# TravisWheelerLab/AvxWindowFmIndex

Measured on AMD Instinct MI355X. Metric: Mkmers/sec located, GRCh38 nucleotide index, higher is better.
Workload: dtype u64

## Files before the change

avxwindowfmindex_amd/_lib.py:

```python
import ctypes as C
import os
import subprocess

_HERE = os.path.dirname(os.path.abspath(__file__))
LIB_PATH = os.environ.get("AWFM_LIB_PATH") or os.path.join(_HERE, "libawfmindex_amd.so")
_LIB = None

AwFmAlphabetAmino, AwFmAlphabetDna, AwFmAlphabetRna = 1, 2, 3
AwFmSuccess, AwFmFileReadOkay, AwFmFileWriteOkay = 1, 2, 3
AwFmGeneralFailure = -1
AwFmIllegalPositionError = -6
AwFmUnsupportedVersionError = -2
AwFmFileReadFail = -11

API_SYMBOLS = [
    "awFmCreateIndex", "awFmCreateIndexFromFasta", "awFmDeallocIndex", "awFmWriteIndexToFile",
    "awFmReadIndexFromFile", "awFmCreateKmerSearchList", "awFmDeallocKmerSearchList", "awFmParallelSearchLocate",
    "awFmParallelSearchCount", "awFmFindSearchRangeForString", "awFmReadSequenceFromFile",
    "awFmCreateInitialQueryRange", "awFmCreateInitialQueryRangeFromChar",
    "awFmNucleotideIterativeStepBackwardSearch", "awFmAminoIterativeStepBackwardSearch",
    "awFmFindDatabaseHitPositions", "awFmFindDatabaseHitPositionSingle",
    "awFmGetLocalSequencePositionFromIndexPosition", "awFmNucleotideBacktraceReturnPreviousLetterIndex",
    "awFmAminoBacktraceReturnPreviousLetterIndex", "awFmGetHeaderStringFromSequenceNumber", "awFmSearchRangeLength",
    "awFmReturnCodeIsFailure", "awFmReturnCodeIsSuccess", "awFmGetNumSequences",
]
GPU_SYMBOLS = [
    "awfmGpuDeviceCount", "awfmGpuLastError", "awfmGpuIndexCreate", "awfmGpuIndexDestroy", "awfmGpuIndexAcquire", "awfmGpuIndexAcquireAll",
    "awfmGpuIndexRelease", "awfmGpuIndexDeviceBytes", "awfmGpuIndexDevice", "awfmGpuIndexSetKernel", "awfmGpuIndexSetWide", "awfmGpuIndexIsWide", "awfmGpuLastBatchStatus", "awfmGpuIndexSetDeepSeed", "awfmGpuIndexSetDenseSa", "awfmGpuPinnedBuffer", "awfmGpuLocateHostWindows", "awfmGpuLocateWindow", "awfmGpuAosLock",
    "awfmGpuAosUnlock", "awfmGpuSearch", "awfmGpuSearchHits", "awfmGpuSearchHitsSparse", "awfmGpuIndexSetOrdered", "awfmGpuSearchHitsIsOrdered", "awfmGpuLastOrderedKernelMs", "awfmGpuLastOrderedKernelIsLookup", "awfmGpuLastOrderedKept",
    "awfmGpuScanScratchBytes", "awfmGpuHitOffsets", "awfmGpuHitOffsetsFromCounts", "awfmGpuLocate", "awfmGpuCountHost", "awfmGpuLocateHost",
    "awfmGpuCreateIndex", "awfmGpuSearchTally", "awfmGpuSynthText", "awfmGpuSynthRandomQueries", "awfmGpuSynthPlantedQueries",
    "awfmGpuSynthMixedLengths", "awfmGpuSynthMixedQueries", "awfmGpuSynthGenomeText", "awfmGpuSynthPlantedQueriesClean",
    "awfmPackKmers", "awfmGpuPackKmers", "awfmGpuUnpackKmers", "awfmGpuHostAlloc", "awfmGpuHostFree", "awfmGpuStreamPacked",
    "awfmGpuStreamChars", "awfmGpuCountPackedHost", "awfmGpuLocatePackedHost", "awfmGpuIndexSetPairImage", "awfmGpuIndexHasPairImage",
    "awfmGpuSearchHitsPacked", "awfmGpuLocateTo", "awfmGpuSearchHitsLineTally", "awfmGpuIndexDeepSeedK", "awfmGpuSearchHitsCompact", "awfmGpuCompactHits", "awfmGpuSortHits",
    "awfmGpuStreamPackedSparse", "awfmGpuStreamCharsSparse", "awfmGpuSearchHitsInOrder", "awfmGpuSearchHitsInOrderCounts",
    "awfmGpuSortHitsOnDevice", "awfmGpuHitOffsetsOnDevice", "awfmGpuLocateOnDevice", "awfmGpuLastOrderedSearchKernelMs", "awfmGpuOrderedKernelLog", "awfmGpuIndexDeepSeedBuildSeconds", "awfmGpuIndexDeepSeedTransientBytes", "awfmGpuIndexHasDenseSa", "awfmGpuIndexDenseSaBuildSeconds", "awfmGpuIndexLengthTableBytes", "awfmGpuIndexLengthTableBuildSeconds", "awfmGpuMixedLookupLineTally",
    "awfmGpuListLocateOnDevice", "awfmGpuLastLookupFront", "awfmGpuLastSearchWasExactLookup", "awfmGpuSynthPlantedQueriesUnique", "awfmGpuStreamRetire", "awfmGpuIndexDescribe", "awfmGpuIndexDeepSeedAllocSeconds", "awfmGpuAosLastStages", "awfmHostCopyGBs",
    "awfmLocalPositions", "awfmGpuIndexSetRecordTable", "awfmGpuIndexNumRecords", "awfmGpuLocalPositions", "awfmGpuLocateHostLocal",
    "awfmLongestSuffixMatches", "awfmGpuLongestSuffixMatches", "awfmOneSubstitutionSearch", "awfmGpuOneSubstitutionSearch",
    "awfmReadCandidates", "awfmGpuReadCandidates", "awfmGpuReadCandidatesScratchBytes",
    "awfmReadChains", "awfmGpuReadChains", "awfmGpuReadChainsScratchBytes",
    "awfmGpuIndexSetText", "awfmGpuIndexTextLength", "awfmTextWindows", "awfmGpuTextWindows", "awfmVerifyChains", "awfmGpuVerifyChains",
    "awfmAlignChains", "awfmGpuAlignChainsScratchBytes", "awfmGpuAlignChains",
    "awfmGpuOrderBuckets", "awfmGpuOrderKmers", "awfmGpuSearchOrderedRecords", "awfmGpuSearchOrderedRecordsCounts", "awfmGpuSearchGeneralRecords", "awfmGpuMergeBucketRuns",
]
CHUNK_SINK = C.CFUNCTYPE(C.c_int, C.c_void_p, C.c_uint64, C.c_uint64, C.POINTER(C.c_uint32), C.POINTER(C.c_uint64), C.c_uint64)


SPARSE_CHUNK_SINK = C.CFUNCTYPE(C.c_int, C.c_void_p, C.c_uint64, C.c_uint64, C.c_uint64, C.POINTER(C.c_uint32), C.POINTER(C.c_uint64),
                                C.POINTER(C.c_uint64), C.c_uint64)
HIT_WINDOW_SINK = C.CFUNCTYPE(C.c_int, C.c_void_p, C.c_uint64, C.c_uint64, C.c_uint64, C.c_uint64, C.POINTER(C.c_uint64))


class AwFmIndexConfiguration(C.Structure):
    _fields_ = [("suffixArrayCompressionRatio", C.c_uint8), ("kmerLengthInSeedTable", C.c_uint8),
                ("alphabetType", C.c_int), ("keepSuffixArrayInMemory", C.c_bool), ("storeOriginalSequence", C.c_bool)]


class AwFmCompressedSuffixArray(C.Structure):
    _fields_ = [("valueBitWidth", C.c_uint8), ("values", C.POINTER(C.c_uint8)), ("compressedByteLength", C.c_uint64)]

# ... 92 lines not shown
        "awFmCreateInitialQueryRange": (AwFmSearchRange, [IP, C.c_char_p, u64]),
        "awFmCreateInitialQueryRangeFromChar": (AwFmSearchRange, [IP, C.c_char]),
        "awFmNucleotideIterativeStepBackwardSearch": (None, [IP, RP, C.c_uint8]),
        "awFmAminoIterativeStepBackwardSearch": (None, [IP, RP, C.c_uint8]),
        "awFmFindDatabaseHitPositions": (C.POINTER(u64), [IP, RP, C.POINTER(C.c_int)]),
        "awFmFindDatabaseHitPositionSingle": (u64, [IP, u64, C.POINTER(C.c_int)]),
        "awFmNucleotideBacktraceReturnPreviousLetterIndex": (C.c_uint8, [IP, C.POINTER(u64)]),
        "awFmAminoBacktraceReturnPreviousLetterIndex": (C.c_uint8, [IP, C.POINTER(u64)]),
        "awFmGetLocalSequencePositionFromIndexPosition": (C.c_int, [IP, C.c_size_t, C.POINTER(C.c_size_t),
                                                                   C.POINTER(C.c_size_t)]),
        "awFmGetHeaderStringFromSequenceNumber": (C.c_int, [IP, C.c_size_t, C.POINTER(C.c_char_p), C.POINTER(C.c_size_t)]),
        "awFmSearchRangeLength": (C.c_size_t, [RP]),
        "awFmReturnCodeIsFailure": (C.c_bool, [C.c_int]),
        "awFmReturnCodeIsSuccess": (C.c_bool, [C.c_int]),
        "awFmGetNumSequences": (C.c_uint32, [IP]),
        "awfmGpuDeviceCount": (C.c_int, []),
        "awfmGpuLastError": (C.c_char_p, []),
        "awfmGpuIndexCreate": (C.c_int, [IP, C.c_int, C.POINTER(vp)]),
        "awfmGpuIndexDestroy": (None, [vp]),
        "awfmGpuIndexAcquire": (vp, [IP]),
        "awfmGpuIndexAcquireAll": (C.c_int, [IP, C.POINTER(vp), C.c_int]),
        "awfmGpuIndexRelease": (None, [IP]),
        "awfmGpuIndexDeviceBytes": (u64, [vp]),
        "awfmGpuIndexDevice": (C.c_int, [vp]),
        "awfmGpuIndexSetKernel": (None, [vp, C.c_int]),
        "awfmGpuIndexSetWide": (None, [vp, C.c_int]),
        "awfmGpuIndexIsWide": (C.c_int, [vp]),
        "awfmGpuLastBatchStatus": (C.c_int, []),
        "awfmGpuIndexSetOrdered": (None, [vp, C.c_int]),
        "awfmGpuSearchHitsIsOrdered": (C.c_int, [vp, C.c_int, C.c_uint32, u64]),
        "awfmGpuLastOrderedKernelMs": (C.c_double, [vp]),
        "awfmGpuLastOrderedKernelIsLookup": (C.c_int, [vp]),
        "awfmGpuLastOrderedKept": (C.c_uint64, [vp]),
        "awfmGpuIndexSetDeepSeed": (C.c_int, [vp, C.c_uint]),
        "awfmGpuIndexSetDenseSa": (C.c_int, [vp, C.c_int]),
        "awfmGpuIndexSetPairImage": (C.c_int, [vp, C.c_int]),
        "awfmGpuIndexHasPairImage": (C.c_int, [vp]),
        "awfmGpuIndexDeepSeedK": (C.c_uint, [vp]),
        "awfmGpuIndexDeepSeedBuildSeconds": (C.c_double, [vp]),
        "awfmGpuIndexDeepSeedTransientBytes": (u64, [vp]),
        "awfmGpuIndexHasDenseSa": (C.c_int, [vp]),
        "awfmGpuIndexDenseSaBuildSeconds": (C.c_double, [vp]),
        "awfmGpuIndexLengthTableBytes": (u64, [vp]),
        "awfmGpuIndexLengthTableBuildSeconds": (C.c_double, [vp]),
        "awfmGpuMixedLookupLineTally": (C.c_int, [vp, vp, vp, u64, C.POINTER(u64 * 8)]),
        "awfmGpuSearch": (C.c_int, [vp, vp, vp, C.c_uint32, u64, vp, vp, vp]),
        "awfmGpuSearchHits": (C.c_int, [vp, vp, vp, C.c_uint32, u64, vp, vp, vp]),
        "awfmGpuSearchHitsSparse": (C.c_int, [vp, vp, vp, C.c_uint32, u64, vp, vp, vp]),
        "awfmGpuSearchHitsCompact": (C.c_int, [vp, vp, vp, C.c_uint32, u64, C.c_int, vp, vp, C.c_uint32, vp, vp]),
        "awfmGpuCompactHits": (C.c_int, [vp, vp, vp, u64, vp, vp, vp, vp, C.c_uint32, vp, vp]),
        "awfmGpuSearchHitsInOrder": (C.c_int, [vp, vp, vp, C.c_uint32, u64, C.c_int, vp, vp, vp]),
        "awfmGpuSearchHitsInOrderCounts": (C.c_int, [vp, vp, vp, C.c_uint32, u64, C.c_int, vp, vp, vp, vp]),
        "awfmGpuOrderBuckets": (C.c_uint32, [vp, C.c_uint32, u64]),
        "awfmGpuOrderKmers": (C.c_int, [vp, vp, C.c_uint32, u64, u64, u64, vp, vp, vp]),
        "awfmGpuSearchOrderedRecords": (C.c_int, [vp, vp, vp, C.c_uint32, C.c_uint32, C.c_uint32, u64, vp, vp, vp]),
        "awfmGpuSearchOrderedRecordsCounts": (C.c_int, [vp, vp, vp, C.c_uint32, C.c_uint32, C.c_uint32, u64, vp, vp, vp, vp]),
        "awfmGpuMergeBucketRuns": (C.c_int, [vp, vp, vp, vp, C.c_uint32, C.c_uint32, C.c_uint32, C.c_uint32, vp, vp, vp]),
        "awfmGpuSearchGeneralRecords": (C.c_int, [vp, vp, C.c_uint32, u64, u64, u64, vp, vp, vp, vp, vp]),
        "awfmGpuSortHits": (C.c_int, [vp, vp, vp, C.c_uint32, vp]),
        "awfmGpuSortHitsOnDevice": (C.c_int, [vp, vp, vp, C.c_uint32, vp, u64, vp]),
        "awfmGpuListLocateOnDevice": (C.c_int, [vp, vp, vp, C.c_uint32, vp, u64, vp, vp, vp, u64, vp, vp]),
        "awfmGpuLastLookupFront": (C.c_int, [vp]),
        "awfmGpuLastSearchWasExactLookup": (C.c_int, [vp]),
        "awfmGpuStreamRetire": (None, [vp, vp]),
        "awfmGpuIndexDescribe": (C.c_int, [vp, C.c_char_p, C.c_int]),
        "awfmGpuIndexDeepSeedAllocSeconds": (C.c_double, [vp]),
# ... 83 lines not shown
```

avxwindowfmindex_amd/api.py:

```python
import ctypes as C
import os

import numpy as np

from . import _lib
from ._lib import (AwFmAlphabetAmino, AwFmAlphabetDna, AwFmAlphabetRna, AwFmFileReadOkay, AwFmFileWriteOkay,
                   AwFmIllegalPositionError, AwFmSuccess, AwFmUnsupportedVersionError)

ILLEGAL_SEQUENCE = 0xFFFFFFFF


class AwFmError(RuntimeError):
    def __init__(self, what, rc):
        msg = _lib.lib().awfmGpuLastError().decode(errors="replace")
        super().__init__(f"{what} failed with AwFmReturnCode {rc}" + (f": {msg}" if msg else ""))
        self.rc = rc


def _check(what, rc, ok=(AwFmSuccess, AwFmFileReadOkay, AwFmFileWriteOkay)):
    if rc not in ok:
        raise AwFmError(what, rc)
    return rc


# ... 915 lines not shown

    def list_locate_on_device(self, d_hit_kmers, d_hit_ranges, capacity, d_num_hits, n, d_sorted_kmers, d_sorted_ranges, d_hit_offsets,
                              capacity_hits, d_positions, stream=0):
        _check("awfmGpuListLocateOnDevice", _lib.lib().awfmGpuListLocateOnDevice(
            self.handle, d_hit_kmers, d_hit_ranges, capacity, d_num_hits, n, d_sorted_kmers, d_sorted_ranges, d_hit_offsets,
            capacity_hits, d_positions or None, stream or None))

    def hit_offsets_on_device(self, d_counts, d_ranges, n, d_hit_offsets, d_scratch, stream=0):
        _check("awfmGpuHitOffsetsOnDevice", _lib.lib().awfmGpuHitOffsetsOnDevice(self.handle, d_counts or None, d_ranges or None, n,
                                                                                 d_hit_offsets, d_scratch, stream or None))

    def locate_on_device(self, d_ranges, d_hit_offsets, n, capacity_hits, d_positions, stream=0):
        _check("awfmGpuLocateOnDevice", _lib.lib().awfmGpuLocateOnDevice(self.handle, d_ranges, d_hit_offsets, n, capacity_hits,
                                                                         d_positions, stream or None))

    def ordered_kernel_log(self, max_entries=1024):
        front = (C.c_double * max_entries)()
        kern = (C.c_double * max_entries)()
        n = _lib.lib().awfmGpuOrderedKernelLog(self.handle, front, kern, max_entries)
        return [(front[i], kern[i]) for i in range(n)]

    def last_ordered_search_kernel_ms(self):
        return float(_lib.lib().awfmGpuLastOrderedSearchKernelMs(self.handle))

    def search_hits_is_ordered(self, has_offsets, fixed_length, n):
        return bool(_lib.lib().awfmGpuSearchHitsIsOrdered(self.handle, int(bool(has_offsets)), fixed_length, n))

    def last_ordered_kernel_ms(self):
        return float(_lib.lib().awfmGpuLastOrderedKernelMs(self.handle))

    def last_ordered_kept(self):
        return int(_lib.lib().awfmGpuLastOrderedKept(self.handle))

    def last_ordered_kernel_is_lookup(self):
        return bool(_lib.lib().awfmGpuLastOrderedKernelIsLookup(self.handle))

    def set_ordered(self, mode):
        _lib.lib().awfmGpuIndexSetOrdered(self.handle, mode)

    def search_tally(self, d_chars, d_offsets, fixed_length, n):
        out = (C.c_uint64 * 4)()
        _check("awfmGpuSearchTally", _lib.lib().awfmGpuSearchTally(self.handle, d_chars, d_offsets or None, fixed_length,
                                                                   n, C.byref(out)))
        return {"seeded": int(out[0]), "steps": int(out[1]), "blocks": int(out[2]), "chars": int(out[3])}

    def search_hits_line_tally(self, d_chars, d_offsets, fixed_length, n):
        out = (C.c_uint64 * 8)()
        _check("awfmGpuSearchHitsLineTally", _lib.lib().awfmGpuSearchHitsLineTally(self.handle, d_chars, d_offsets or None,
                                                                                   fixed_length, n, C.byref(out)))
        keys = ("seed_table_lines", "deep_table_lines", "pair_level_lines", "nuc_level_lines", "ordered_kmers",
                "record_bytes_per_kmer", "kmers_with_hits", "general_kmers")
        return {k: int(v) for k, v in zip(keys, out)}

    def hit_offsets(self, d_ranges, n, d_hit_offsets, d_scratch, stream=0):
        total = C.c_uint64(0)
        _check("awfmGpuHitOffsets", _lib.lib().awfmGpuHitOffsets(self.handle, d_ranges, n, d_hit_offsets, d_scratch,
                                                                 C.byref(total), stream or None))
        return int(total.value)

    def hit_offsets_from_counts(self, d_counts, n, d_hit_offsets, d_scratch, stream=0):
        total = C.c_uint64(0)
        _check("awfmGpuHitOffsetsFromCounts", _lib.lib().awfmGpuHitOffsetsFromCounts(
            self.handle, d_counts, n, d_hit_offsets, d_scratch, C.byref(total), stream or None))
        return int(total.value)

    def locate(self, d_ranges, d_hit_offsets, n, total_hits, d_positions, stream=0):
# ... 23 lines not shown
```

avxwindowfmindex_amd/csrc/awfm_gpu_ordered.hip:

```cpp
#include <cstring>
#include <cstdio>
#include <cstdlib>
#include <cstddef>

#include <hip/hip_runtime.h>
#include <hip/hip_ext.h>
#include <rocprim/rocprim.hpp>

#include "awfm_ordered_kernel.h"
#include "awfm_amino_lookup_kernel.h"
#include "awfm_count_order_kernel.h"

namespace {

inline size_t alignUp256(size_t v) { return (v + 255) / 256 * 256; }

__global__ void __launch_bounds__(256) fillSparseKernel(unsigned *__restrict__ kmers, ulonglong2 *__restrict__ ranges, unsigned cap,
                                                        unsigned *__restrict__ count) {
  const unsigned i = blockIdx.x * 256u + threadIdx.x;
  if (i < cap) {
    kmers[i] = 0xFFFFFFFFu;
    ranges[i] = make_ulonglong2(1ull, 0ull);
  }
  if (i == 0) *count = 0u;
// ... 233 lines not shown
    (void)hipGetLastError();
    return false;
  }
  return alive * 4u < g->orderSamples;
}

extern "C" int awfmGpuLastOrderedKernelIsLookup(AwFmGpuIndex *g) {
  if (!g) return 0;
  std::lock_guard<std::mutex> lock(g->orderMutex);
  return lastSearchLookedUpFirst(g) ? 1 : 0;
}

extern "C" uint64_t awfmGpuLastOrderedKept(AwFmGpuIndex *g) {
  if (!g) return 0;
  std::lock_guard<std::mutex> lock(g->orderMutex);
  if (!g->orderKeptAt) return 0;
  DeviceGuard guard(g->device);
  unsigned kept = 0;
  if (hipDeviceSynchronize() != hipSuccess || hipMemcpy(&kept, g->orderKeptAt, sizeof kept, hipMemcpyDeviceToHost) != hipSuccess) {
    (void)hipGetLastError();
    return 0;
  }
  if (g->orderLookupFused && g->orderFusedKeptAt && lastSearchLookedUpFirst(g)) {
    unsigned words[kFusedCounters * 16u];
    if (hipMemcpy(words, g->orderFusedKeptAt, sizeof words, hipMemcpyDeviceToHost) != hipSuccess) {
      (void)hipGetLastError();
      return 0;
    }
    uint64_t total = kept;
    for (unsigned i = 0; i < kFusedCounters; i++) total += words[i * 16u];
    return total;
  }
  return kept;
}

extern "C" double awfmGpuLastOrderedKernelMs(AwFmGpuIndex *g) {
  if (!g) return -1.0;
  std::lock_guard<std::mutex> lock(g->orderMutex);
  const bool front = lastSearchLookedUpFirst(g);
  if (front ? !g->orderTimedFront : !g->orderTimedKernel) return -1.0;
  hipEvent_t from = g->orderTiming[front ? 0 : 2], to = g->orderTiming[front ? 1 : 3];
  if (!from || !to) return -1.0;
  float ms = 0.0f;
  if (hipEventSynchronize(to) != hipSuccess || hipEventElapsedTime(&ms, from, to) != hipSuccess) return -1.0;
  return (double)ms;
}

extern "C" int awfmGpuOrderedKernelLog(AwFmGpuIndex *g, double *frontMs, double *kernelMs, int max) {
  if (!g || !frontMs || !kernelMs || max <= 0) return 0;
  std::lock_guard<std::mutex> lock(g->orderMutex);
  DeviceGuard guard(g->device);
  unsigned long long n = g->orderLogCount;
  if (n > AwFmGpuIndex::kOrderLogMax) n = AwFmGpuIndex::kOrderLogMax;
  if (n > (unsigned long long)max) n = (unsigned long long)max;
  for (unsigned long long i = 0; i < n; i++) {
    const AwFmGpuIndex::OrderLogEntry &e = g->orderLog[(g->orderLogCount - n + i) % AwFmGpuIndex::kOrderLogMax];
    float ms = 0.0f;
    frontMs[i] = e.front && hipEventSynchronize(e.ev[1]) == hipSuccess && hipEventElapsedTime(&ms, e.ev[0], e.ev[1]) == hipSuccess ? (double)ms : -1.0;
    kernelMs[i] = e.kernel && hipEventSynchronize(e.ev[3]) == hipSuccess && hipEventElapsedTime(&ms, e.ev[2], e.ev[3]) == hipSuccess ? (double)ms : -1.0;
  }
  (void)hipGetLastError();
  g->orderLogCount = 0;
  return (int)n;
}

extern "C" double awfmGpuLastOrderedSearchKernelMs(AwFmGpuIndex *g) {
// ... 321 lines not shown
      hipLaunchKernelGGL(fillNoHitKernel, dim3((unsigned)g->numCUs * 8u), dim3(256), 0, s,
                         rangesOfHitsOnly && dCounts ? (ulonglong2 *)nullptr : rng, dCounts, nq);
      BUCKET_TRY(hipGetLastError());
    }
    g->orderSampleAt = (const unsigned *)aliveOut;
    if (front == kFrontBoth) sampleAlive = (const unsigned *)aliveOut;
    else {
      bySample = false;
      lookupFirst = front == kFrontLookupOnly;
    }
  } else {
    BUCKET_TRY(hipMemsetAsync(w, 0, startAt, s));
    BUCKET_TRY(fillSparseList(sparse, s));
    if (!sparse) {
      hipLaunchKernelGGL(fillNoHitKernel, dim3((unsigned)g->numCUs * 8u), dim3(256), 0, s,
                         rangesOfHitsOnly && dCounts ? (ulonglong2 *)nullptr : rng, dCounts, nq);
      BUCKET_TRY(hipGetLastError());
    }
    bySample = false;
    g->orderSampleAt = (const unsigned *)(w + kSampleAt);
  }
  const bool lookupOnly = prepFused && front == kFrontLookupOnly;
  g->orderLookup = bySample ? 2 : (lookupFirst ? 1 : 0);
  g->orderSamples = kSamples;
  g->orderKeptAt = lookupOnly ? generalCount : bucketStart + bins;
  g->orderTimedFront = false;
  if (lookupFirst || bySample) {
    const bool timed = g->orderTiming[0] != nullptr;
    g->orderLookupFused = true;
    g->orderFusedKeptAt = (const unsigned *)(w + kKeptAt);
    {
      const bool pairOff = !pairSteps(g);
      const bool superInLds = !pairOff && narrow && awfmPairSuperInLds(g);
      DevIndex dev = g->image->dev;
      dev.pairSuperInLds = superInLds ? 1u : 0u;
      const size_t lds = superInLds ? (size_t)g->image->dev.numPairSuper * 64u : 0u;
      const unsigned perCU = narrow ? 7u : 6u;
      unsigned fusedGrid = (unsigned)(perShare256 * kShares < (unsigned long long)g->numCUs * perCU ? perShare256 * kShares : (unsigned long long)g->numCUs * perCU);
      fusedGrid = (fusedGrid + kShares - 1u) / kShares * kShares;
      {
        const unsigned long long tripsPerShare = (shareSize(nq) + 1023ull) / 1024ull, groupsPerShare = fusedGrid / kShares;
        if (groupsPerShare > 0u && tripsPerShare > groupsPerShare) {
          const unsigned long long tripsEach = (tripsPerShare + groupsPerShare - 1ull) / groupsPerShare;
          if (tripsEach <= 64ull) fusedGrid = (unsigned)((tripsPerShare + tripsEach - 1ull) / tripsEach) * kShares;
        }
      }
#define AWFM_LOOKUP_GO(NR)                                                                                                               \
  launchLookupSearchAt<32u, NR>(fixedLength, fusedGrid, lds, s, dev, dChars, fmt, useNext | (pairOff ? 2u : 0u) | (lookupOnly ? 4u : 0u), nq, \
                                (unsigned long long *)(w + codesAt), lookupOnly ? (unsigned *)recs : numbers, lookupOnly ? generalCount : shareCount, \
                                hist, binsPad, sampleAlive, kSamples, rng, dCounts, sparse ? *sparse : SparseOut(),                      \
                                (unsigned *)(w + kKeptAt), timed ? g->orderTiming[0] : nullptr, timed ? g->orderTiming[1] : nullptr)
      if (narrow) AWFM_LOOKUP_GO(true);
      else AWFM_LOOKUP_GO(false);
#undef AWFM_LOOKUP_GO
    }
    g->orderTimedFront = timed;
    if (timed) g->orderLog[(g->orderLogCount - 1u) % AwFmGpuIndex::kOrderLogMax].front = true;
    BUCKET_TRY(hipGetLastError());
  }
  if (lookupOnly) {
    enum AwFmReturnCode rc = AwFmSuccess;
    if (!packed)
      rc = narrow ? launchLeftover<true, false>(g, s, dChars, nullptr, fixedLength, nq, rng, dCounts, recs, 8u, 0u, generalCount, sparse)
                  : launchLeftover<false, false>(g, s, dChars, nullptr, fixedLength, nq, rng, dCounts, recs, 8u, 0u, generalCount, sparse);
    if (rc != AwFmSuccess) return -(int)rc;
    BUCKET_TRY(slotScope.end());
    return 1;
  }
  if (lookupFirst) {
  } else if (packed)
    hipLaunchKernelGGL((encodeCodesKernel<true>), dim3(encodeGrid), dim3(256), bins * 4u, s, dChars, fixedLength, fmt, nq,
                       (unsigned long long *)nullptr, hist, binsPad);
  else
    launchEncode4(fixedLength, encodeGrid, bins * 4u, s, dChars, fmt, nq, (unsigned long long *)(w + codesAt), hist, binsPad, sampleAlive, kSamples);
  BUCKET_TRY(hipGetLastError());
  hipLaunchKernelGGL(bucketScanSharesKernel, dim3(1), dim3(1024), 0, s, hist, bins, binsPad, bucketStart, generalCount, (unsigned)nq);
  BUCKET_TRY(hipGetLastError());
  const size_t partitionLds = (size_t)kPartitionTile * 8u + 3u * binsPad * 4u;
  static std::once_flag ldsOnce;
  static hipError_t ldsError = hipSuccess;
  std::call_once(ldsOnce, [] {
// ... 1120 lines not shown
```

avxwindowfmindex_amd/csrc/awfm_ordered_kernel.h:

```cpp
#ifndef AWFM_ORDERED_KERNEL_H
#define AWFM_ORDERED_KERNEL_H

#include "awfm_search_kernel.h"
#include "awfm_pair.h"

namespace {

__device__ __forceinline__ void decodeWord(unsigned word, unsigned &packed, unsigned &badBits) {
  unsigned t = (word >> 1) & 0x03030303u;
  t ^= (t >> 1) & 0x01010101u;
  const unsigned b0 = t & 0x01010101u, b1 = (t >> 1) & 0x01010101u, b01 = b0 & b1;
  const unsigned expect = 0x61616161u + (b0 << 1) + b1 * 6u + b01 * 11u;
  unsigned diff = ((word | 0x20202020u) ^ expect) & ~b01;
  diff |= diff >> 4;
  diff |= diff >> 2;
  diff |= diff >> 1;
  diff &= 0x01010101u;
  badBits = (diff & 1u) | ((diff >> 7) & 2u) | ((diff >> 14) & 4u) | ((diff >> 21) & 8u);
  packed = ((t & 3u) << 6) | ((t >> 4) & 0x30u) | ((t >> 14) & 0x0Cu) | (t >> 24);
}

__device__ __forceinline__ void decodeWordAny(unsigned word, unsigned countMask, unsigned &packed, unsigned &diffs) {
  unsigned t = (word >> 1) & 0x03030303u;
  t ^= (t >> 1) & 0x01010101u;
// ... 227 lines not shown
  const bool LIST = sparse.count != nullptr;
  __shared__ unsigned long long sC[24];
  __shared__ unsigned sMask[(kBlockMask + 1) * kSlices];
  __shared__ unsigned long long sSuper[NARROW ? 1 : kMaxNucSuper * 4];
  __shared__ unsigned long long sPairC[16];
  extern __shared__ unsigned sPairSuper[];
  __shared__ unsigned long long sCodes[4][kFusedSlots];
  __shared__ unsigned sNum[4][kFusedSlots];
  __shared__ pos_t sSp[4][kFusedSlots], sEp[4][kFusedSlots];
  constexpr unsigned kHitBuffer = 32;
  __shared__ unsigned sHitKmers[4][kHitBuffer];
  __shared__ unsigned long long sHitRanges[4][kHitBuffer][2];
  __shared__ unsigned sHitLeft[4], sWavesDone;
  if (!lookupChosen(sampleAlive, samples, true)) return;
  if (threadIdx.x == 0) sWavesDone = 0u;
  if (threadIdx.x < 24) sC[threadIdx.x] = ix.prefixSums[threadIdx.x];
  stageMaskTable(sMask);
  nucStageSuper<NARROW>(ix, sSuper);
  if (PAIR) pairStageTables<NARROW, 16u>(ix, sPairC, sPairSuper);
  __syncthreads();
  const unsigned bins = (1u << f.bucketBits) + 1u;
  constexpr unsigned kLoads = (K + 1u + 3u) / 4u;
  const unsigned shift = (unsigned)((unsigned long long)chars & 3ull);
  typedef const Dwords4 __attribute__((address_space(1))) *GlobalDwords4;
  const unsigned share = blockIdx.x % kShares, localBlock = blockIdx.x / kShares, localGrid = gridDim.x / kShares;
  const unsigned long long size = shareSize(numQueries), first = size * share;
  const unsigned long long last = first + size < numQueries ? first + size : numQueries;
  const unsigned long long tableMask = (1ull << (2u * f.depth)) - 1ull;
  const unsigned lengthBits = deepLengthBits(ix);
  const unsigned lane = threadIdx.x & 63u, gl = threadIdx.x % G, firstSlice = gl;
  const unsigned w = (unsigned)__builtin_amdgcn_readfirstlane((int)(threadIdx.x >> 6));
  unsigned blockBase = 0, blockUsed = 0, blockSlots = 0;
  unsigned hitFill = 0, keptHere = 0;
  auto flushHits = [&]() {
    if (hitFill != 0u) {
      __builtin_amdgcn_fence(__ATOMIC_RELEASE, "wavefront");
      __builtin_amdgcn_wave_barrier();
      unsigned listBase = 0;
      if (lane == 0) listBase = atomicAdd(sparse.count, hitFill);
      listBase = (unsigned)__builtin_amdgcn_readfirstlane((int)listBase);
      if (lane < hitFill && listBase + lane < sparse.cap) {
        sparse.kmers[listBase + lane] = sHitKmers[w][lane];
        sparse.ranges[listBase + lane] = make_ulonglong2(sHitRanges[w][lane][0], sHitRanges[w][lane][1]);
      }
      __builtin_amdgcn_wave_barrier();
      hitFill = 0;
    }
  };
  const unsigned long long waveFirst = first + 4ull * ((unsigned long long)localBlock * 256ull + (threadIdx.x & ~63u));
  for (unsigned long long tw = waveFirst; tw < last; tw += 4ull * localGrid * 256ull) {
    const unsigned long long t = tw + 4ull * lane;
    unsigned long long codes[4];
    unsigned bad[4];
    if (t * K + 16ull * kLoads <= numQueries * K) {
      const GlobalDwords4 from = (GlobalDwords4)(((unsigned long long)chars + t * K) & ~3ull);
      unsigned dw[kLoads * 4u + 1u];
#pragma unroll
      for (unsigned j = 0; j < kLoads; j++) {
        const Dwords4 q = from[j];
        dw[4u * j] = q.x;
        dw[4u * j + 1u] = q.y;
        dw[4u * j + 2u] = q.z;
        dw[4u * j + 3u] = q.w;
      }
      dw[kLoads * 4u] = 0u;
      unsigned al[K + 1u];
// ... 53 lines not shown
      amask[i] = __ballot(append[i]);
      abefore[i] = atotal;
      atotal += (unsigned)__popcll(amask[i]);
    }
    if (atotal != 0u && (useNext & 4u) != 0u) {
      unsigned base = 0;
      if (lane == 0) base = atomicAdd(shareCount, atotal);
      base = (unsigned)__builtin_amdgcn_readfirstlane((int)base);
#pragma unroll
      for (unsigned i = 0; i < 4u; i++)
        if (append[i]) {
          const unsigned long long rec = numQueries - 1ull - (base + abefore[i] + (unsigned)__popcll(amask[i] & ((1ull << lane) - 1ull)));
          ((unsigned long long *)numbersOut)[rec] = (unsigned long long)(t + i);
        }
    } else if (atotal != 0u) {
      if (blockUsed + atotal > blockSlots) {
        if (blockUsed + lane < blockSlots) codesOut[first + blockBase + blockUsed + lane] = kCodeNone;
        blockSlots = atotal > kLookupBlock || tw + 256ull > last ? atotal : kLookupBlock;
        unsigned base = 0;
        if (lane == 0) base = atomicAdd(&shareCount[share * kShareCountStride], blockSlots);
        blockBase = (unsigned)__builtin_amdgcn_readfirstlane((int)base);
        blockUsed = 0;
      }
#pragma unroll
      for (unsigned i = 0; i < 4u; i++)
        if (append[i]) {
          const unsigned long long slot = first + blockBase + blockUsed + abefore[i] + (unsigned)__popcll(amask[i] & ((1ull << lane) - 1ull));
          codesOut[slot] = bad[i] ? kCodeGeneral : codes[i];
          numbersOut[slot] = (unsigned)(t + i);
          atomicAdd(&hist[share * binsPad + (bad[i] ? bins - 1u : bucketOf(f, codes[i]))], 1u);
        }
      blockUsed += atotal;
    }
    const unsigned inBatch = stotal < kFusedSlots ? stotal : kFusedSlots;
    keptHere += inBatch;
    if (inBatch != 0u) {
      __builtin_amdgcn_fence(__ATOMIC_RELEASE, "wavefront");
      __builtin_amdgcn_wave_barrier();
      __builtin_amdgcn_fence(__ATOMIC_ACQUIRE, "wavefront");
      for (unsigned pass = 0; pass < inBatch; pass += 64u / G) {
        const unsigned slot = pass + lane / G;
        const bool live = slot < inBatch;
        pos_t sp = 1, ep = 0;
        unsigned long long rem = 0;
        unsigned index = 0;
        int pos = -1;
        if (live) {
          const unsigned long long c = sCodes[w][slot];
          index = sNum[w][slot];
          sp = sSp[w][slot];
          ep = sEp[w][slot];
          rem = c >> (2u * f.depth);
          pos = (int)(K - f.depth) - 1;
        }
        if (PAIR) {
          while (pos >= 1 && sp <= ep) {
            const unsigned c2 = (unsigned)rem & 3u, c1 = (unsigned)(rem >> 2) & 3u;
            if (pairSearchStep<NARROW>(ix, sPairC, sPairSuper, sMask, gl, c1 * 4u + c2, sp, ep) == kPairFlagged) {
              nucFastStep<G, NARROW>(ix, sC, sSuper, sMask, firstSlice, c2, sp, ep);
              if (sp <= ep) nucFastStep<G, NARROW>(ix, sC, sSuper, sMask, firstSlice, c1, sp, ep);
            }
            pos -= 2;
            rem >>= 4;
          }
          if (pos == 0 && sp <= ep) {
            nucFastStep<G, NARROW>(ix, sC, sSuper, sMask, firstSlice, (unsigned)rem & 3u, sp, ep);
            pos--;
          }
        } else {
          while (pos >= 0 && sp <= ep) {
            nucFastStep<G, NARROW>(ix, sC, sSuper, sMask, firstSlice, (unsigned)rem & 3u, sp, ep);
            pos--;
            rem >>= 2;
          }
        }
        const bool hit = live && gl == 0 && sp <= ep;
        if (LIST) {
          const unsigned long long hitMask = __ballot(hit);
          if (hitMask != 0ull) {
            const unsigned hits = (unsigned)__builtin_amdgcn_readfirstlane((int)__popcll(hitMask));
            if (hit) {
              const unsigned at = hitFill + (unsigned)__popcll(hitMask & ((1ull << lane) - 1ull));
              sHitKmers[w][at] = index;
              sHitRanges[w][at][0] = (unsigned long long)sp;
              sHitRanges[w][at][1] = (unsigned long long)ep;
            }
            hitFill = (unsigned)__builtin_amdgcn_readfirstlane((int)(hitFill + hits));
          }
          if (hitFill + 64u / G > kHitBuffer) flushHits();
        } else if (hit) {
          if (ranges) ranges[index] = make_ulonglong2((unsigned long long)sp, (unsigned long long)ep);
          if (counts) counts[index] = (unsigned)(ep - sp + (pos_t)1);
        }
      }
      __builtin_amdgcn_wave_barrier();
    }
  }
  for (unsigned at = blockUsed + lane; at < blockSlots; at += 64u) codesOut[first + blockBase + at] = kCodeNone;
  if (lane == 0 && keptHere) atomicAdd(&keptCounters[((blockIdx.x * 4u + w) % kFusedCounters) * 16u], keptHere);
  if (LIST) {
    if (lane == 0) sHitLeft[w] = hitFill;
    __builtin_amdgcn_fence(__ATOMIC_RELEASE, "workgroup");
    unsigned arrived = 0;
    if (lane == 0) arrived = atomicAdd(&sWavesDone, 1u);
    arrived = (unsigned)__builtin_amdgcn_readfirstlane((int)arrived);
    if (arrived == 3u) {
      __builtin_amdgcn_fence(__ATOMIC_ACQUIRE, "workgroup");
      unsigned total = 0;
      for (unsigned v = 0; v < 4u; v++) total += sHitLeft[v];
      if (total != 0u) {
        unsigned listBase = 0;
        if (lane == 0) listBase = atomicAdd(sparse.count, total);
        listBase = (unsigned)__builtin_amdgcn_readfirstlane((int)listBase);
        unsigned before = 0;
        for (unsigned v = 0; v < 4u; v++) {
          const unsigned n = sHitLeft[v];
          if (lane < n && listBase + before + lane < sparse.cap) {
            sparse.kmers[listBase + before + lane] = sHitKmers[v][lane];
            sparse.ranges[listBase + before + lane] = make_ulonglong2(sHitRanges[v][lane][0], sHitRanges[v][lane][1]);
          }
          before += n;
        }
      }
    }
  }
}

template <bool AMINO>
__global__ void __launch_bounds__(256)
    lookupPrepKernel(const DevIndex ix, const unsigned char *__restrict__ chars, const unsigned fixedLen, const unsigned depth,
                     const unsigned useNext, const unsigned long long numQueries, const unsigned samples,
                     unsigned long long *__restrict__ aliveOut, unsigned long long *__restrict__ aliveNext,
// ... 897 lines not shown
```

include/awfm_gpu.h:

```cpp
#ifndef AWFM_GPU_H
#define AWFM_GPU_H

#include "AwFmIndex.h"

#ifdef __cplusplus
extern "C" {
#endif

typedef struct AwFmGpuIndex AwFmGpuIndex;

enum AwFmGpuKernel {
  AWFM_GPU_KERNEL_AUTO = 0,
  AWFM_GPU_KERNEL_GROUP8 = 1,
  AWFM_GPU_KERNEL_GROUP4 = 2,
  AWFM_GPU_KERNEL_GROUP2 = 3,
  AWFM_GPU_KERNEL_GROUP1 = 4
};

int awfmGpuDeviceCount(void);
const char *awfmGpuLastError(void);
enum AwFmReturnCode awfmGpuLastBatchStatus(void);


enum AwFmReturnCode awfmGpuIndexCreate(const struct AwFmIndex *index, int device, AwFmGpuIndex **out);
// ... 179 lines not shown

#define AWFM_ALIGN_MAX_LENGTH (1u << 16)
#define AWFM_ALIGN_MAX_OPS 4096u
#define AWFM_ALIGN_OVERHANG 0xFFFFFFFBu
struct AwFmAlignOutputs {
  uint32_t *editDistances;
  uint64_t *textBegins;
  uint64_t *textEnds;
  uint32_t *numOps;
  uint32_t *ops;
  uint64_t *numUnaligned;
  uint64_t *numTruncated;
};
enum AwFmReturnCode awfmAlignChains(const struct AwFmVerifyInputs *in, const uint32_t *slots, uint64_t numReads, uint32_t maxCandidates,
                                    uint32_t bandPad, uint32_t maxDrift, uint32_t maxOps, const uint8_t *text, uint64_t length,
                                    const uint64_t *sequenceEnds, uint64_t numRecords, enum AwFmAlphabetType alphabet,
                                    const struct AwFmAlignOutputs *out, unsigned threads);
uint64_t awfmGpuAlignChainsScratchBytes(const AwFmGpuIndex *g, uint32_t maxRows);
enum AwFmReturnCode awfmGpuAlignChains(AwFmGpuIndex *g, const struct AwFmVerifyInputs *dIn, const uint32_t *dSlots, uint64_t numReads,
                                       uint32_t maxCandidates, uint32_t bandPad, uint32_t maxDrift, uint32_t maxOps, uint32_t maxRows,
                                       const struct AwFmAlignOutputs *dOut, void *dScratch, void *stream);

void awfmGpuIndexSetOrdered(AwFmGpuIndex *g, int mode);
int awfmGpuSearchHitsIsOrdered(const AwFmGpuIndex *g, int hasOffsets, uint32_t fixedLength, uint64_t numQueries);
void awfmGpuStreamRetire(AwFmGpuIndex *g, void *stream);

double awfmGpuLastOrderedKernelMs(AwFmGpuIndex *g);
int awfmGpuLastOrderedKernelIsLookup(AwFmGpuIndex *g);
int awfmGpuLastLookupFront(AwFmGpuIndex *g);
int awfmGpuLastSearchWasExactLookup(AwFmGpuIndex *g);
double awfmGpuLastOrderedSearchKernelMs(AwFmGpuIndex *g);
int awfmGpuOrderedKernelLog(AwFmGpuIndex *g, double *frontMs, double *kernelMs, int max);
uint64_t awfmGpuLastOrderedKept(AwFmGpuIndex *g);

enum AwFmReturnCode awfmGpuSearchTally(AwFmGpuIndex *g, const uint8_t *dChars, const uint64_t *dOffsets,
                                       uint32_t fixedLength, uint64_t numQueries, uint64_t tallyOut[4]);

enum AwFmReturnCode awfmGpuMixedLookupLineTally(AwFmGpuIndex *g, const uint8_t *dChars, const uint64_t *dOffsets,
                                                uint64_t numQueries, uint64_t tallyOut[8]);

enum AwFmReturnCode awfmGpuSearchHitsLineTally(AwFmGpuIndex *g, const uint8_t *dChars, const uint64_t *dOffsets,
                                               uint32_t fixedLength, uint64_t numQueries, uint64_t tallyOut[8]);

uint64_t awfmGpuScanScratchBytes(uint64_t numQueries);
enum AwFmReturnCode awfmGpuHitOffsets(AwFmGpuIndex *g, const struct AwFmSearchRange *dRanges, uint64_t numQueries,
                                      uint64_t *dHitOffsets, void *dScratch, uint64_t *totalHits, void *stream);
enum AwFmReturnCode awfmGpuHitOffsetsFromCounts(AwFmGpuIndex *g, const uint32_t *dCounts, uint64_t numQueries,
                                                uint64_t *dHitOffsets, void *dScratch, uint64_t *totalHits, void *stream);

enum AwFmReturnCode awfmGpuHitOffsetsOnDevice(AwFmGpuIndex *g, const uint32_t *dCounts, const struct AwFmSearchRange *dRanges,
                                              uint64_t numQueries, uint64_t *dHitOffsets, void *dScratch, void *stream);
enum AwFmReturnCode awfmGpuLocateOnDevice(AwFmGpuIndex *g, const struct AwFmSearchRange *dRanges, const uint64_t *dHitOffsets,
                                          uint64_t numQueries, uint64_t capacityHits, uint64_t *dPositions, void *stream);

enum AwFmReturnCode awfmGpuLocate(AwFmGpuIndex *g, const struct AwFmSearchRange *dRanges,
                                  const uint64_t *dHitOffsets, uint64_t numQueries, uint64_t totalHits,
                                  uint64_t *dPositions, void *stream);

enum AwFmReturnCode awfmGpuLocateTo(AwFmGpuIndex *g, const struct AwFmSearchRange *dRanges,
                                    const uint64_t *dHitOffsets, uint64_t numQueries, uint64_t totalHits,
                                    uint64_t *dPositions, uint64_t *outPositions, void *stream);

enum AwFmReturnCode awfmGpuLocateWindow(AwFmGpuIndex *g, const struct AwFmSearchRange *dRanges, const uint64_t *dHitOffsets,
                                        uint64_t queryBegin, uint64_t queryEnd, uint64_t hitBegin, uint64_t hitEnd,
                                        uint64_t *dPositions, uint64_t *outPositions, void *stream);

// ... 104 lines not shown
```

Before: 36410.

## Add adaptive second-window deep-seed filter before backward search in fused lookup kernel

Before the per-kmer backward search in the fused lookup kernel, each kept kmer is checked against the deep-seed table a second time, using a later window of its code. Kmers whose second window has no occurrence are dropped, and the survivors are compacted in LDS so the search loop runs over fewer slots. An adaptive gate turns the test off when it rarely drops anything, and it also rechecks every sixteenth trip. The change adds tested and dropped counters and a host query that reads them back. The cost is an extra random table load plus wave barriers on each batch.

```diff
diff --git a/avxwindowfmindex_amd/_lib.py b/avxwindowfmindex_amd/_lib.py
--- a/avxwindowfmindex_amd/_lib.py
+++ b/avxwindowfmindex_amd/_lib.py
@@ -27,7 +27,7 @@
 GPU_SYMBOLS = [
     "awfmGpuDeviceCount", "awfmGpuLastError", "awfmGpuIndexCreate", "awfmGpuIndexDestroy", "awfmGpuIndexAcquire", "awfmGpuIndexAcquireAll",
     "awfmGpuIndexRelease", "awfmGpuIndexDeviceBytes", "awfmGpuIndexDevice", "awfmGpuIndexSetKernel", "awfmGpuIndexSetWide", "awfmGpuIndexIsWide", "awfmGpuLastBatchStatus", "awfmGpuIndexSetDeepSeed", "awfmGpuIndexSetDenseSa", "awfmGpuPinnedBuffer", "awfmGpuLocateHostWindows", "awfmGpuLocateWindow", "awfmGpuAosLock",
-    "awfmGpuAosUnlock", "awfmGpuSearch", "awfmGpuSearchHits", "awfmGpuSearchHitsSparse", "awfmGpuIndexSetOrdered", "awfmGpuSearchHitsIsOrdered", "awfmGpuLastOrderedKernelMs", "awfmGpuLastOrderedKernelIsLookup", "awfmGpuLastOrderedKept",
+    "awfmGpuAosUnlock", "awfmGpuSearch", "awfmGpuSearchHits", "awfmGpuSearchHitsSparse", "awfmGpuIndexSetOrdered", "awfmGpuSearchHitsIsOrdered", "awfmGpuLastOrderedKernelMs", "awfmGpuLastOrderedKernelIsLookup", "awfmGpuLastOrderedKept", "awfmGpuLastSecondWindow",
     "awfmGpuScanScratchBytes", "awfmGpuHitOffsets", "awfmGpuHitOffsetsFromCounts", "awfmGpuLocate", "awfmGpuCountHost", "awfmGpuLocateHost",
     "awfmGpuCreateIndex", "awfmGpuSearchTally", "awfmGpuSynthText", "awfmGpuSynthRandomQueries", "awfmGpuSynthPlantedQueries",
     "awfmGpuSynthMixedLengths", "awfmGpuSynthMixedQueries", "awfmGpuSynthGenomeText", "awfmGpuSynthPlantedQueriesClean",
@@ -186,6 +186,7 @@
         "awfmGpuLastOrderedKernelMs": (C.c_double, [vp]),
         "awfmGpuLastOrderedKernelIsLookup": (C.c_int, [vp]),
         "awfmGpuLastOrderedKept": (C.c_uint64, [vp]),
+        "awfmGpuLastSecondWindow": (None, [vp, C.POINTER(C.c_uint64 * 2)]),
         "awfmGpuIndexSetDeepSeed": (C.c_int, [vp, C.c_uint]),
         "awfmGpuIndexSetDenseSa": (C.c_int, [vp, C.c_int]),
         "awfmGpuIndexSetPairImage": (C.c_int, [vp, C.c_int]),
diff --git a/avxwindowfmindex_amd/api.py b/avxwindowfmindex_amd/api.py
--- a/avxwindowfmindex_amd/api.py
+++ b/avxwindowfmindex_amd/api.py
@@ -971,6 +971,11 @@
     def last_ordered_kept(self):
         return int(_lib.lib().awfmGpuLastOrderedKept(self.handle))
 
+    def last_second_window(self):
+        out = (C.c_uint64 * 2)()
+        _lib.lib().awfmGpuLastSecondWindow(self.handle, C.byref(out))
+        return int(out[0]), int(out[1])
+
     def last_ordered_kernel_is_lookup(self):
         return bool(_lib.lib().awfmGpuLastOrderedKernelIsLookup(self.handle))
 
diff --git a/avxwindowfmindex_amd/csrc/awfm_gpu_ordered.hip b/avxwindowfmindex_amd/csrc/awfm_gpu_ordered.hip
--- a/avxwindowfmindex_amd/csrc/awfm_gpu_ordered.hip
+++ b/avxwindowfmindex_amd/csrc/awfm_gpu_ordered.hip
@@ -289,6 +289,24 @@
     return total;
   }
   return kept;
+}
+
+extern "C" void awfmGpuLastSecondWindow(AwFmGpuIndex *g, uint64_t out[2]) {
+  if (!out) return;
+  out[0] = out[1] = 0;
+  if (!g) return;
+  std::lock_guard<std::mutex> lock(g->orderMutex);
+  if (!g->orderLookupFused || !g->orderFusedKeptAt || !lastSearchLookedUpFirst(g)) return;
+  DeviceGuard guard(g->device);
+  unsigned words[kFusedCounters * 16u];
+  if (hipDeviceSynchronize() != hipSuccess || hipMemcpy(words, g->orderFusedKeptAt, sizeof words, hipMemcpyDeviceToHost) != hipSuccess) {
+    (void)hipGetLastError();
+    return;
+  }
+  for (unsigned i = 0; i < kFusedCounters; i++) {
+    out[0] += words[i * 16u + 1u];
+    out[1] += words[i * 16u + 2u];
+  }
 }
 
 extern "C" double awfmGpuLastOrderedKernelMs(AwFmGpuIndex *g) {
@@ -676,6 +694,8 @@
     {
       const bool pairOff = !pairSteps(g);
       const bool superInLds = !pairOff && narrow && awfmPairSuperInLds(g);
+      unsigned secondBits = 0u;
+      if (const char *env = awfmGpuDiag("second_window")) secondBits = atoi(env) == 0 ? 8u : 32u;
       DevIndex dev = g->image->dev;
       dev.pairSuperInLds = superInLds ? 1u : 0u;
       const size_t lds = superInLds ? (size_t)g->image->dev.numPairSuper * 64u : 0u;
@@ -690,7 +710,7 @@
         }
       }
 #define AWFM_LOOKUP_GO(NR)                                                                                                               \
-  launchLookupSearchAt<32u, NR>(fixedLength, fusedGrid, lds, s, dev, dChars, fmt, useNext | (pairOff ? 2u : 0u) | (lookupOnly ? 4u : 0u), nq, \
+  launchLookupSearchAt<32u, NR>(fixedLength, fusedGrid, lds, s, dev, dChars, fmt, useNext | (pairOff ? 2u : 0u) | (lookupOnly ? 4u : 0u) | secondBits, nq, \
                                 (unsigned long long *)(w + codesAt), lookupOnly ? (unsigned *)recs : numbers, lookupOnly ? generalCount : shareCount, \
                                 hist, binsPad, sampleAlive, kSamples, rng, dCounts, sparse ? *sparse : SparseOut(),                      \
                                 (unsigned *)(w + kKeptAt), timed ? g->orderTiming[0] : nullptr, timed ? g->orderTiming[1] : nullptr)
diff --git a/avxwindowfmindex_amd/csrc/awfm_ordered_kernel.h b/avxwindowfmindex_amd/csrc/awfm_ordered_kernel.h
--- a/avxwindowfmindex_amd/csrc/awfm_ordered_kernel.h
+++ b/avxwindowfmindex_amd/csrc/awfm_ordered_kernel.h
@@ -283,6 +283,10 @@
   const unsigned w = (unsigned)__builtin_amdgcn_readfirstlane((int)(threadIdx.x >> 6));
   unsigned blockBase = 0, blockUsed = 0, blockSlots = 0;
   unsigned hitFill = 0, keptHere = 0;
+  const unsigned secondW = f.depth + ((useNext & 1u) != 0u ? 2u : 0u);
+  const bool second = K > secondW && (useNext & 8u) == 0u, forceSecond = (useNext & 32u) != 0u;
+  const unsigned secondShift = second ? 2u * (K - secondW) : 0u;
+  unsigned gateTested = 0, gateDropped = 0, testedHere = 0, droppedHere = 0, trip = 0;
   auto flushHits = [&]() {
     if (hitFill != 0u) {
       __builtin_amdgcn_fence(__ATOMIC_RELEASE, "wavefront");
@@ -402,12 +406,56 @@
         }
       blockUsed += atotal;
     }
-    const unsigned inBatch = stotal < kFusedSlots ? stotal : kFusedSlots;
+    unsigned inBatch = stotal < kFusedSlots ? stotal : kFusedSlots;
     keptHere += inBatch;
+    trip++;
     if (inBatch != 0u) {
       __builtin_amdgcn_fence(__ATOMIC_RELEASE, "wavefront");
       __builtin_amdgcn_wave_barrier();
       __builtin_amdgcn_fence(__ATOMIC_ACQUIRE, "wavefront");
+      if (second && (forceSecond || (stotal <= kFusedSlots && (gateTested < 64u || 2u * gateDropped >= gateTested || (trip & 15u) == 0u)))) {
+        bool passes = false;
+        unsigned long long c = 0;
+        if (lane < inBatch) {
+          c = sCodes[w][lane];
+          const unsigned long long window = c >> secondShift;
+          const uint2 e = ((const uint2 *)ix.deepSeed)[window & tableMask];
+          passes = (e.y & lengthBits) != 0u &&
+                   ((useNext & 1u) == 0u || ((e.y >> (16u + ((unsigned)(window >> (2u * f.depth)) & 15u))) & 1u) != 0u);
+        }
+        const unsigned long long passMask = __ballot(passes);
+        const unsigned passed = (unsigned)__popcll(passMask);
+        if (passed != inBatch) {
+          unsigned num = 0;
+          pos_t sp = 0, ep = 0;
+          if (passes) {
+            num = sNum[w][lane];
+            sp = sSp[w][lane];
+            ep = sEp[w][lane];
+          }
+          __builtin_amdgcn_fence(__ATOMIC_ACQUIRE, "wavefront");
+          __builtin_amdgcn_wave_barrier();
+          if (passes) {
+            const unsigned rank = (unsigned)__popcll(passMask & ((1ull << lane) - 1ull));
+            sCodes[w][rank] = c;
+            sNum[w][rank] = num;
+            sSp[w][rank] = sp;
+            sEp[w][rank] = ep;
+          }
+          __builtin_amdgcn_fence(__ATOMIC_RELEASE, "wavefront");
+          __builtin_amdgcn_wave_barrier();
+          __builtin_amdgcn_fence(__ATOMIC_ACQUIRE, "wavefront");
+        }
+        testedHere += inBatch;
+        droppedHere += inBatch - passed;
+        gateTested += inBatch;
+        gateDropped += inBatch - passed;
+        if (gateTested >= 4096u) {
+          gateTested >>= 1;
+          gateDropped >>= 1;
+        }
+        inBatch = passed;
+      }
       for (unsigned pass = 0; pass < inBatch; pass += 64u / G) {
         const unsigned slot = pass + lane / G;
         const bool live = slot < inBatch;
@@ -468,6 +516,8 @@
   }
   for (unsigned at = blockUsed + lane; at < blockSlots; at += 64u) codesOut[first + blockBase + at] = kCodeNone;
   if (lane == 0 && keptHere) atomicAdd(&keptCounters[((blockIdx.x * 4u + w) % kFusedCounters) * 16u], keptHere);
+  if (lane == 0 && testedHere) atomicAdd(&keptCounters[((blockIdx.x * 4u + w) % kFusedCounters) * 16u + 1u], testedHere);
+  if (lane == 0 && droppedHere) atomicAdd(&keptCounters[((blockIdx.x * 4u + w) % kFusedCounters) * 16u + 2u], droppedHere);
   if (LIST) {
     if (lane == 0) sHitLeft[w] = hitFill;
     __builtin_amdgcn_fence(__ATOMIC_RELEASE, "workgroup");
diff --git a/include/awfm_gpu.h b/include/awfm_gpu.h
--- a/include/awfm_gpu.h
+++ b/include/awfm_gpu.h
@@ -235,6 +235,7 @@
 double awfmGpuLastOrderedSearchKernelMs(AwFmGpuIndex *g);
 int awfmGpuOrderedKernelLog(AwFmGpuIndex *g, double *frontMs, double *kernelMs, int max);
 uint64_t awfmGpuLastOrderedKept(AwFmGpuIndex *g);
+void awfmGpuLastSecondWindow(AwFmGpuIndex *g, uint64_t out[2]);
 
 enum AwFmReturnCode awfmGpuSearchTally(AwFmGpuIndex *g, const uint8_t *dChars, const uint64_t *dOffsets,
                                        uint32_t fixedLength, uint64_t numQueries, uint64_t tallyOut[4]);
```

Measured after the change: 37710 (median of 6 runs). +3.6%, better.
